# Ryan21wy/HSIMAE

Measured on AMD Instinct MI355X. Metric: HSI patches/sec (9x9x96, mask 75%) pretrain fwd+bwd, higher is better.
Workload: dtype bf16; 1 GPU; HSIMAE-Base pretrain fwd+bwd, 9x9x96 cubes, per-GPU batch 4096, mask 0.75, bf16 MFMA operands / fp32 accumulate + residual; per_gpu_batch=4096, global_batch=4096, parallelism=dp1

## Files before the change

### hsimae_amd/_lib.py

```python
from __future__ import annotations

import ctypes as C
import os

HERE = os.path.dirname(os.path.abspath(__file__))
LIB_PATH = os.environ.get("HSIMAE_LIB") or os.path.join(HERE, "libhsimae_hip.so")

i32, i64, f32, vp = C.c_int32, C.c_int64, C.c_float, C.c_void_p


class Config(C.Structure):
    _fields_ = [("bands", i32), ("embed_dim", i32), ("depth", i32), ("s_depth", i32), ("num_heads", i32),
                ("dec_dim", i32), ("dec_depth", i32), ("dec_heads", i32), ("hidden", i32), ("dec_hidden", i32),
                ("norm_pix_loss", i32), ("precision", i32)]


class IO(C.Structure):
    _fields_ = [("x", vp), ("sn", i64), ("sb", i64), ("sh", i64), ("sw", i64),
                ("N", i32), ("len_t", i32), ("len_l", i32),
                ("noise1", vp), ("noise2", vp), ("params", vp), ("wpk", vp),
                ("workspace", vp), ("workspace_bytes", i64),
                ("grad_scale", f32), ("want_recons", i32),
                ("loss", vp), ("pred_img", vp), ("mask_img", vp), ("mask", vp),
                ("ids_keep", vp), ("ids_restore", vp), ("latent", vp), ("pred", vp), ("drop_scale", vp),
# ... 87 lines not shown
class SceneParams(C.Structure):
    _fields_ = [("scene", vp), ("scene_f64", i32), ("H", i32), ("W", i32), ("C", i32),
                ("p0", i64), ("pixels", vp), ("N", i32),
                ("out", vp), ("sn", i64), ("sb", i64), ("sh", i64), ("sw", i64)]


class SceneBatchParams(C.Structure):
    _fields_ = [("scene", vp), ("scene_f64", i32), ("H", i32), ("W", i32), ("C", i32),
                ("items", vp), ("N", i32), ("n_items", i64), ("pixels", vp), ("labels", vp), ("flips", vp),
                ("out", vp), ("sn", i64), ("sb", i64), ("sh", i64), ("sw", i64), ("y", vp), ("bad", vp)]


class GwpcaParams(C.Structure):
    _fields_ = [("scene", vp), ("scene_f64", i32), ("H", i32), ("W", i32), ("C", i32), ("nc", i32), ("group", i32), ("whiten", i32),
                ("minmax", vp), ("mean", vp), ("lambda_", vp), ("proj", vp), ("group_off", vp)]


class ClsParams(C.Structure):
    _fields_ = [("logits", vp), ("ld", i32), ("targets", vp), ("N", i32), ("C", i32), ("ignore_index", i64), ("first", i32),
                ("loss", vp), ("n_valid", vp), ("dlogits", vp), ("ldd", i32), ("pred", vp), ("bad", vp), ("workspace", vp)]


class ClassProbParams(C.Structure):
    _fields_ = [("logits", vp), ("ld", i32), ("N", i32), ("C", i32), ("first", i32), ("view", i32), ("n_views", i32),
                ("acc", vp), ("lda", i32), ("H", i32), ("W", i32), ("p0", i64), ("pixels", vp),
                ("label_map", vp), ("conf_map", vp), ("margin_map", vp), ("probs", vp), ("ldp", i32)]


class RowNormalizeParams(C.Structure):
    _fields_ = [("x", vp), ("ld", i32), ("N", i32), ("D", i32), ("out", vp), ("ldo", i32), ("norms", vp)]
# ... 68 lines not shown
    "hsimae_dec_block_fwd": (C.c_int, [C.POINTER(DecBlockWeights), vp, vp, vp, vp, vp, i32, i32, i32, vp]),
    "hsimae_dec_block_bwd": (C.c_int, [C.POINTER(DecBlockWeights), C.POINTER(DecBlockGrads), vp, vp, vp, vp, vp, vp, vp, i32, i32, vp, vp]),
    "hsimae_attn_fwd": (C.c_int, [C.POINTER(AttnParams), vp]),
    "hsimae_attn_bwd": (C.c_int, [C.POINTER(AttnParams), vp]),
    "hsimae_attn_block_fwd": (C.c_int, [C.POINTER(AttnBlockWeights), vp, vp, vp, vp, vp, vp, vp, i32, i32, i32, i32, i32, i32, vp]),
    "hsimae_attn_block_bwd": (C.c_int, [C.POINTER(AttnBlockWeights), vp, vp, vp, vp, vp, vp, vp, vp, vp, vp, vp, vp, i32, i32, i32,
                                        i32, i32, i32, i32, vp]),
    "hsimae_wgrad": (C.c_int, [C.POINTER(WgradParams), vp]),
    "hsimae_wgrad_msplit": (i32, [i32, i64]),
    "hsimae_ln_bwd": (C.c_int, [C.POINTER(LnBwdParams), vp]),
    "hsimae_ln_fwd": (C.c_int, [vp, vp, vp, vp, i32, i32, vp]),
    "hsimae_assemble_fwd": (C.c_int, [C.POINTER(AssembleParams), vp]),
    "hsimae_assemble_bwd": (C.c_int, [C.POINTER(AssembleParams), vp]),
    "hsimae_loss_partials": (C.c_int, [i32, i32]),
    "hsimae_loss": (C.c_int, [C.POINTER(LossParams), vp]),
    "hsimae_adamw_step": (C.c_int, [vp, vp, vp, vp, vp, i64, f32, f32, f32, f32, f32, i32, vp]),
    "hsimae_grad_norm": (C.c_int, [C.POINTER(GradSeg), i32, f32, i32, i32, f32, f32, vp, vp, vp]),
    "hsimae_adamw_step_ctl": (C.c_int, [vp, vp, vp, vp, vp, i32, i64, f32, f32, f32, f32, f32, vp, vp]),
    "hsimae_adamw_step_groups": (C.c_int, [vp, vp, vp, vp, vp, i32, i64, C.POINTER(AdamWGroup), i32, f32, f32, f32, i32, vp, vp]),
    "hsimae_lamb_step": (C.c_int, [vp, vp, vp, vp, vp, i32, i64, vp, i32, i32, C.POINTER(AdamWGroup), i32, f32, f32, f32, f32, i32,
                                   vp, vp, vp, vp, vp]),
    "hsimae_ema_update": (C.c_int, [vp, vp, i64, C.c_double, i32, i32, vp, vp]),
    "hsimae_ema_swap": (C.c_int, [vp, vp, i64, vp]),
    "hsimae_cube_gather": (C.c_int, [C.POINTER(CubeParams), vp]),
    "hsimae_scene_windows": (C.c_int, [C.POINTER(SceneParams), vp]),
    "hsimae_class_argmax": (C.c_int, [C.POINTER(SceneParams), vp, i32, i32, i32, vp, vp]),
    "hsimae_scene_batch": (C.c_int, [C.POINTER(SceneBatchParams), vp]),
    "hsimae_gwpca_workspace_bytes": (i64, [C.POINTER(GwpcaParams)]),
    "hsimae_gwpca_fit": (C.c_int, [C.POINTER(GwpcaParams), vp, vp]),
    "hsimae_gwpca_apply": (C.c_int, [C.POINTER(GwpcaParams), vp, i32, vp]),
# ... 77 lines not shown
```

### hsimae_amd/build.py

```python
from __future__ import annotations

import os
import subprocess
import sys
from concurrent.futures import ThreadPoolExecutor

HERE = os.path.dirname(os.path.abspath(__file__))
CSRC = os.path.join(HERE, "csrc")
LIB = os.path.join(HERE, "libhsimae_hip.so")
UNITS = ["gemm", "attn", "attn_wide", "wgrad", "elem", "pack", "fused_dec", "fused_enc", "loader", "scene", "gwpca", "cls", "clip", "lamb", "ema", "prob", "knn", "api"]
HIPCC = os.environ.get("HIPCC", "/opt/rocm/bin/hipcc")
BASE_FLAGS = ["--offload-arch=gfx950", "-O3", "-fPIC", "-std=c++17", "-Wno-unused-value", "-fvisibility=hidden"]
FLAGS = BASE_FLAGS + os.environ.get("HSIMAE_HIPCC_EXTRA", "").split()


def flags_hash(flags: list[str]) -> str:
    import hashlib
    return hashlib.sha256(" ".join(flags).encode()).hexdigest()[:16]


def unit_flags(unit: str, flags: list[str]) -> list[str]:
    if unit != "api":
        return list(flags)
    return list(flags) + [f"-DHS_BUILD_FLAGS_HASH=0x{flags_hash(flags)}ULL", f"-DHS_BUILD_DEFAULT_FLAGS={int(flags == BASE_FLAGS)}",
                          f"-DHS_KERNEL_SOURCE_HASH=0x{kernel_source_hash()}ULL"]
# ... 100 lines not shown
```

### hsimae_amd/csrc/api.hip

```cpp
#include "common.h"
#include "kernels.h"
#include "plan.h"
#include <vector>
#include <algorithm>
#include <cstring>
#include <cstdlib>
#include <mutex>
#include <unordered_map>
#include <initializer_list>

using namespace hsplan;

namespace {

#define CK(expr) do { int _e = (expr); if (_e) return _e; } while (0)
#define CK0(expr) do { int _e0 = (expr); if (_e0) return _e0; } while (0)

inline hipStream_t S(void* s) { return reinterpret_cast<hipStream_t>(s); }
struct BlkP : BlockW {
    struct I8 { const uint8_t* w; const uint8_t* s; } qkv8, p8, w1_8, w3_8, w2_8, qkvT8, pT8, w13T8, w2T8;
};

BlkP resolve(const BlkOff& o, const BlkW& w, const float* P, const hs_bf16* wpk, const WLayout& WL, int h) {
    const float* fbase = reinterpret_cast<const float*>(wpk + WL.bf16_elems);
// ... 17 lines not shown
    if (!off("HSIMAE_FUSED_DEC")) b |= SC_FUSED_DEC;
    if (!off("HSIMAE_DEC_SPLIT")) b |= SC_DEC_SPLIT;
    if (one("HSIMAE_FP8_UNFUSED")) b |= SC_FP8_UNFUSED;
    if (!off("HSIMAE_FUSED_MLP")) b |= SC_FUSED_MLP;
    if (!off("HSIMAE_FUSED_ATTN_BLOCK")) b |= SC_ATTN_BLOCK;
    if (!off("HSIMAE_FUSED_ATTN_BLOCK256")) b |= SC_ATTN_BLOCK256;
    if (!off("HSIMAE_FUSED_ATTN_BLOCK_BWD")) b |= SC_ATTN_BLOCK_BWD;
    if (!off("HSIMAE_FUSED_PROJ_BWD")) b |= SC_PROJ_BWD;
    if (!off("HSIMAE_FUSED_LNBWD")) b |= SC_LNBWD;
    if (!off("HSIMAE_FUSED_LNBWD_512")) b |= SC_LNBWD_512;
    if (!off("HSIMAE_ATTN_BWD_RECOMPUTE")) b |= SC_RECOMPUTE;
    if (!off("HSIMAE_WGRAD_SLAB")) b |= SC_WGRAD_SLAB;
    if (!off("HSIMAE_DEC_SLAB")) b |= SC_DEC_SLAB;
    if (!off("HSIMAE_WGRAD_PLANAR")) b |= SC_PLANAR;
    if (!off("HSIMAE_FUSED_ATTN_BLOCK256_BWD")) b |= SC_ATTN_BLOCK256_BWD;
    return b;
}
struct SchedRec { uint32_t enc = 0, dec = 0; bool has_enc = false, has_dec = false; uint64_t gen = 0; };
std::mutex g_sched_mu;
std::unordered_map<const void*, SchedRec> g_sched;
uint64_t g_sched_gen = 0;
void record_sched(const void* ws, bool enc, bool dec, uint32_t bits) {
    std::lock_guard<std::mutex> lk(g_sched_mu);
    if (g_sched.size() > 4096 && g_sched.find(ws) == g_sched.end()) {
        std::vector<uint64_t> gens;
        gens.reserve(g_sched.size());
        for (auto& kv : g_sched) gens.push_back(kv.second.gen);
        std::nth_element(gens.begin(), gens.begin() + gens.size() / 2, gens.end());
        const uint64_t cut = gens[gens.size() / 2];
        for (auto it = g_sched.begin(); it != g_sched.end();) it = it->second.gen < cut ? g_sched.erase(it) : std::next(it);
// ... 283 lines not shown
        if (!io->workspace || !io->params || !io->wpk) return HSIMAE_ENULL;
        if (reinterpret_cast<uintptr_t>(io->workspace) % 256) return HSIMAE_EALIGN;
        carve(c.g, c.N, c.K, reinterpret_cast<char*>(io->workspace), c.w);
        if (c.w.bytes > io->workspace_bytes) return HSIMAE_EDIMS;
    }
    return HSIMAE_OK;
}

BlockPlan enc_plan(const Ctx& c, uint32_t sc) {
    return plan_block(c.g.D, c.g.H, c.g.h, c.K, c.N, c.Me, enc_linears_fp8(c.g.prec, c.g.D, sc), sc);
}
BlockPlan dec_block_plan(const Ctx& c, uint32_t sc) {
    return plan_block(c.g.Dd, c.g.Hd, c.g.hdec, c.g.TL, c.N, c.Md, false, sc);
}

int decoder_stack_fwd(const Ctx& c, const hsimae_io* io, uint32_t sc, float* pred, hipStream_t s) {
    const Geo& g = c.g; const Ws& w = c.w; const float* P = io->params;
    AssembleParams as; std::memset(&as, 0, sizeof(as));
    as.y = w.y; as.N = c.N; as.K = c.K; as.TL = g.TL; as.Dd = g.Dd; as.ld = g.Ddp; as.ids_restore = io->ids_restore; as.pos = P + c.L.dpos;
    as.yfull = w.yfull;
    CK(hs_assemble_fwd(as, s));
    const DecPlan dec = plan_dec(c.g.Dd, c.g.Hd, c.g.hdec, c.g.TL, sc);
    const BlockPlan lay = dec_block_plan(c, sc);
    const float* z = w.yfull;
    for (int i = 0; i < g.ddepth; ++i) {
        const BlkP bp = resolve(c.L.bd[i], c.W.bd[i], P, io->wpk, c.W, g.hdec);
        const BlkBuf& b = w.bd[i];
        if (!dec.fused) {
            CK(block_fwd(bp, lay, z, b, 0, 9, nullptr, s));
        } else if (dec.split) {
            CK(hs_dec_attn_fwd(z, b.x1, b.o, b.lse, c.N, g.TL, bp, s));
            CK(hs_enc_mlp_fwd(b.x1, nullptr, b.x2, (int)c.Md, g.Dd, bp, s));
        } else {
            CK(hs_dec_block_fwd(z, b.x1, b.x2, b.o, b.lse, c.N, g.TL, bp, s));
        }
        z = b.x2;
    }
    GemmParams p = gp();
    p.A = z; p.lda = g.Ddp; p.M = (int)c.Md; p.N = 80; p.K = g.Ddp; p.n_valid = 72; p.W = io->wpk + c.W.dp; p.bias = P + c.L.dpb;
    p.gamma = P + c.L.dnw; p.beta = P + c.L.dnb; p.u_out = w.zn; p.ldu = g.Ddp; p.out = pred; p.ldo = 72; p.ln_width = g.Dd;
    return hs_gemm(p, A_F32_LN, E_F32, s);
}

}

extern "C" unsigned hs_variant_bits_gemm();
extern "C" unsigned hs_variant_bits_attn();
extern "C" unsigned hs_variant_bits_attn_wide();
extern "C" unsigned hs_variant_bits_wgrad();
extern "C" unsigned hs_variant_bits_elem();
extern "C" unsigned hs_variant_bits_pack();
extern "C" unsigned hs_variant_bits_fused_dec();
extern "C" unsigned hs_variant_bits_fused_enc();
extern "C" unsigned hs_variant_bits_loader();
extern "C" unsigned hs_variant_bits_scene();
extern "C" unsigned hs_variant_bits_gwpca();
extern "C" unsigned hs_variant_bits_cls();
extern "C" unsigned hs_variant_bits_clip();
extern "C" unsigned hs_variant_bits_lamb();
extern "C" unsigned hs_variant_bits_ema();
extern "C" unsigned hs_variant_bits_prob();
extern "C" unsigned hs_variant_bits_knn();
#ifndef HS_KERNEL_SOURCE_HASH
#define HS_KERNEL_SOURCE_HASH 0ULL
#endif
#ifndef HS_BUILD_FLAGS_HASH
#define HS_BUILD_FLAGS_HASH 0ULL
#endif
#ifndef HS_BUILD_DEFAULT_FLAGS
#define HS_BUILD_DEFAULT_FLAGS 0
#endif

extern "C" {

int hsimae_version(void) { return HSIMAE_VERSION; }

int hsimae_build_info(hsimae_build_info_t* out) {
    if (!out) return HSIMAE_ENULL;
    out->abi_version = HSIMAE_VERSION;
    out->variant_bits = hs_variant_bits() | hs_variant_bits_gemm() | hs_variant_bits_attn() | hs_variant_bits_attn_wide() | hs_variant_bits_wgrad() | hs_variant_bits_elem() | hs_variant_bits_pack() | hs_variant_bits_fused_dec() | hs_variant_bits_fused_enc() | hs_variant_bits_loader() | hs_variant_bits_scene() | hs_variant_bits_gwpca() | hs_variant_bits_cls() | hs_variant_bits_clip() | hs_variant_bits_lamb() | hs_variant_bits_ema() | hs_variant_bits_prob() | hs_variant_bits_knn();
    out->kernel_source_hash = HS_KERNEL_SOURCE_HASH;
    out->flags_hash = HS_BUILD_FLAGS_HASH;
    out->default_flags = HS_BUILD_DEFAULT_FLAGS;
    out->reserved = 0;
    return HSIMAE_OK;
}
const char* hsimae_variant_name(int bit) {
    switch (bit) {
#define HS_X(b, name) case b: return #name;
        HS_VARIANT_TABLE(HS_X)
#undef HS_X
        default: return nullptr;
    }
}

// ... 42 lines not shown

struct DropRs { const float* a; const float* m; };
static DropRs drop_rs(const hsimae_io* io, int e, int64_t Me) {
    if (!io->drop_scale) return DropRs{nullptr, nullptr};
    const float* base = io->drop_scale + (int64_t)e * 2 * Me;
    return DropRs{base, base + Me};
}

static int forward_impl(const hsimae_config* cfg, const hsimae_io* io, void* stream, bool encoder_only) {
    Ctx c; CK(make_ctx(cfg, io, c, true));
    if (!io->x || !io->noise1 || !io->noise2 || !io->mask || !io->ids_keep || !io->ids_restore) return HSIMAE_ENULL;
    if (encoder_only ? !io->latent : !io->loss) return HSIMAE_ENULL;
    if (!encoder_only && io->want_recons && (!io->pred_img || !io->mask_img)) return HSIMAE_ENULL;
    hipStream_t s = S(stream);
    const Geo& g = c.g; const float* P = io->params; const Ws& w = c.w;
    const uint32_t sc = sched_from_env();
    record_sched(io->workspace, true, !encoder_only, sc);
    const BlockPlan enc = enc_plan(c, sc);

    MaskParams m; m.noise1 = io->noise1; m.noise2 = io->noise2; m.N = c.N; m.T = g.T; m.L = 9; m.len_t = c.len_t;
    m.len_l = c.len_l; m.ids_keep = io->ids_keep; m.ids_restore = io->ids_restore; m.mask = io->mask;
    CK(hs_mask(m, s));
    PatchParams pp; pp.x = io->x; pp.sn = io->sn; pp.sb = io->sb; pp.sh = io->sh; pp.sw = io->sw; pp.N = c.N; pp.T = g.T;
    pp.K = c.K; pp.ids_keep = io->ids_keep; pp.out = w.a_pe; pp.pos_ids = nullptr;
    CK(hs_patch_gather(pp, s));
    GemmParams p = gp();
    p.A = w.a_pe; p.lda = 96; p.M = (int)c.Me; p.N = g.Dp; p.K = 96; p.n_valid = g.D; p.W = io->wpk + c.W.pe; p.bias = P + c.L.peb;
    p.pos = P + c.L.pos; p.ids = io->ids_keep; p.ldpos = g.D; p.out = w.x0; p.ldo = g.Dp;
    CK(hs_gemm(p, A_BF16, E_POS_F32, s));

    const float* x = w.x0;
// ... 25 lines not shown
    }
    for (int i = 0; i < g.nfus; ++i) {
        BlkP bp = resolve(c.L.bf[i], c.W.bf[i], P, io->wpk, c.W, g.h);
        const DropRs rf = drop_rs(io, (g.has_axis ? 2 * g.sdepth : 0) + i, c.Me);
        CK(block_fwd(bp, enc, x, w.bf[i], 0, c.len_l, nullptr, s, rf.a, rf.m));
        x = w.bf[i].x2;
    }
    if (encoder_only) {
        CK(hs_ln_fwd(x, P + c.L.nw, P + c.L.nb, io->latent, (int)c.Me, g.D, s, g.Dp, g.D));
        return HSIMAE_OK;
    }
    p = gp();
    p.A = x; p.lda = g.Dp; p.M = (int)c.Me; p.N = g.Ddp; p.K = g.Dp; p.n_valid = g.Dd; p.W = io->wpk + c.W.de; p.bias = P + c.L.deb;
    p.gamma = P + c.L.nw; p.beta = P + c.L.nb; p.u_out = w.lat; p.ldu = g.Dp; p.out = w.y; p.ldo = g.Ddp; p.ln_width = g.D;
    CK(hs_gemm(p, A_F32_LN, E_F32, s));
    CK(decoder_stack_fwd(c, io, sc, w.pred, s));
    LossParams lp; std::memset(&lp, 0, sizeof(lp));
    const float sum_mask = (float)((int64_t)c.N * (g.TL - c.K));
    lp.x = io->x; lp.sn = io->sn; lp.sb = io->sb; lp.sh = io->sh; lp.sw = io->sw; lp.N = c.N; lp.T = g.T; lp.pred = w.pred;
    lp.mask = io->mask; lp.norm_pix = g.norm_pix; lp.inv_scale = io->grad_scale / (72.f * sum_mask); lp.partial = w.partial;
    lp.loss = io->loss; lp.sum_mask = sum_mask; lp.dpred = w.dpred;
    lp.pred_img = io->want_recons ? io->pred_img : nullptr; lp.mask_img = io->want_recons ? io->mask_img : nullptr;
    CK(hs_loss(lp, s));
    if (io->pred) CK((int)hipMemcpyAsync(io->pred, w.pred, c.Md * 72 * 4, hipMemcpyDeviceToDevice, s));
    if (io->latent) CK(hs_ln_fwd(x, P + c.L.nw, P + c.L.nb, io->latent, (int)c.Me, g.D, s, g.Dp, g.D));
    return HSIMAE_OK;
}

int hsimae_forward(const hsimae_config* cfg, const hsimae_io* io, void* stream) { return forward_impl(cfg, io, stream, false); }
int hsimae_encode(const hsimae_config* cfg, const hsimae_io* io, void* stream) { return forward_impl(cfg, io, stream, true); }

int hsimae_decode(const hsimae_config* cfg, const hsimae_io* io, const float* latent, float* pred, void* stream) {
    Ctx c; CK(make_ctx(cfg, io, c, true));
    if (!latent || !pred || !io->ids_restore) return HSIMAE_ENULL;
    hipStream_t s = S(stream);
    const Geo& g = c.g; const float* P = io->params; const Ws& w = c.w;
    const uint32_t sc = sched_from_env();
    record_sched(io->workspace, false, true, sc);
    GemmParams p = gp();
    const float* lat_in = latent;
    if (g.Dp != g.D) {
        CK((int)hipMemcpy2DAsync(w.G2, (size_t)g.Dp * 4, latent, (size_t)g.D * 4, (size_t)g.D * 4, (size_t)c.Me, hipMemcpyDeviceToDevice, s));
        lat_in = w.G2;
    }
    p.A = lat_in; p.lda = g.Dp; p.M = (int)c.Me; p.N = g.Ddp; p.K = g.Dp; p.n_valid = g.Dd; p.W = io->wpk + c.W.de; p.bias = P + c.L.deb;
    p.out = w.y; p.ldo = g.Ddp;
    CK(hs_gemm(p, A_F32, E_F32, s));
    CK(hs_rows_to_bf16(lat_in, w.lat, c.Me, g.Dp, nullptr, s));
    return decoder_stack_fwd(c, io, sc, pred, s);
}

static int encoder_backward(const Ctx& c, const hsimae_io* io, float* grads, hipStream_t s, Emitter& emit, uint32_t sc) {
// ... 35 lines not shown
        }
        if (!per_block) {
            for (int i = g.sdepth - 1; i >= 0; --i) CK(emit(L.b2[i].n1w, L.b2[i].end, s));
            for (int i = g.sdepth - 1; i >= 0; --i) CK(emit(L.b1[i].n1w, L.b1[i].end, s));
        }
    }
    CK(wgrad_one(w.G0, true, g.Dp, w.a_pe, 96, g.D, 72, c.Me, (g.D + 127) / 128, grads, L.pew, L.peb, io->det_acc, s));
    CK(emit(0, L.peb + g.D, s));
    return HSIMAE_OK;
}

static int decoder_backward(const Ctx& c, const hsimae_io* io, float* grads, hipStream_t s, Emitter& emit, uint32_t sc) {
    const Geo& g = c.g; const float* P = io->params; const Ws& w = c.w; const PLayout& L = c.L;
    const float* zlast = w.bd[g.ddepth - 1].x2;
    GemmParams p = gp();
    p.A = w.dpred; p.lda = 96; p.M = (int)c.Md; p.N = g.Ddp; p.K = 96; p.n_valid = g.Dd; p.W = io->wpk + c.W.dpT; p.out = w.du; p.ldo = g.Ddp;
    CK(hs_gemm(p, A_BF16, E_F32, s));
    CK(wgrad_one(w.dpred, false, 96, w.zn, g.Ddp, 72, g.Dd, c.Md, 1, grads, L.dpw, L.dpb, io->det_acc, s));
    LnBwdParams l; std::memset(&l, 0, sizeof(l));
    l.du = w.du; l.x = zlast; l.gamma = P + L.dnw; l.dres = nullptr; l.dx = w.G0; l.dgamma = grads + L.dnw; l.dbeta = grads + L.dnb;
    l.M = (int)c.Md; l.d = g.Dd; l.ld = g.Ddp; l.det_base = grads; l.det_acc = io->det_acc;
    CK(hs_ln_bwd(l, s));
    CK(emit(L.dnw, L.total, s));

    const DecPlan dec = plan_dec(c.g.Dd, c.g.Hd, c.g.hdec, c.g.TL, sc);
    const BlockPlan lay = dec_block_plan(c, sc);
    for (int i = g.ddepth - 1; i >= 0; --i) {
        BlkP bp = resolve(L.bd[i], c.W.bd[i], P, io->wpk, c.W, g.hdec);
        const float* xin = (i == 0) ? w.yfull : w.bd[i - 1].x2;
        if (dec.fused) {
            DecBlockBwd d;
            d.x = xin; d.x1 = w.bd[i].x1; d.dy = w.G0; d.dx1_tmp = w.G1; d.dx = w.G0; d.o = w.bd[i].o; d.lse = w.bd[i].lse;
            d.nsamples = c.N; d.Ts = g.TL; d.slab = dec.slab ? w.slab : nullptr;
            CK(hs_dec_block_bwd(bp, dec_grads(grads, L.bd[i], HsDet{grads, reinterpret_cast<long long*>(io->det_acc)}), d, s));
        } else {
            CK(block_bwd(bp, lay, L.bd[i], grads, xin, w.bd[i], 0, 9, w.G0, w.sc, w.G0, 0, s, 1, nullptr, nullptr, io->det_acc));
        }
// ... 270 lines not shown
}
int hsimae_lamb_step(float* params, const float* grads, float* exp_avg, float* exp_avg_sq, const uint8_t* group,
                     int32_t group_uniform, int64_t n, const hsimae_lamb_tensor* tensors, int32_t ntensors, int32_t nchunks,
                     const hsimae_adamw_group* table, int32_t ngroups, float beta1, float beta2, float eps, float trust_clip,
                     int32_t always_adapt, double* partials, float* ratios, int32_t* bad, const hsimae_clip_ctl* ctl, void* stream) {
    return hs_lamb_step(params, grads, exp_avg, exp_avg_sq, group, group_uniform, n, tensors, ntensors, nchunks, table, ngroups, beta1,
                        beta2, eps, trust_clip, always_adapt, partials, ratios, bad, ctl, S(stream));
}
int hsimae_ema_update(float* ema, const float* params, int64_t n, double decay, int32_t warmup, int32_t step,
                      const hsimae_clip_ctl* ctl, void* stream) {
    return hs_ema_update(ema, params, n, decay, warmup, step, ctl, S(stream));
}
int hsimae_ema_swap(float* a, float* b, int64_t n, void* stream) { return hs_ema_swap(a, b, n, S(stream)); }
int hsimae_loss_partials(int32_t N, int32_t T) { return hs_loss_partials(N, T); }
int hsimae_loss(const hsimae_loss_params* p, void* stream) { return p ? hs_loss(*p, S(stream)) : HSIMAE_ENULL; }

}
```

### hsimae_amd/csrc/kernels.h

```cpp
#pragma once
#include "common.h"
#include "../../include/hsimae_hip.h"

enum AKind { A_BF16 = HSIMAE_A_BF16, A_F32 = HSIMAE_A_F32, A_F32_LN = HSIMAE_A_F32_LN };
enum Epi { E_BF16 = HSIMAE_E_BF16, E_F32 = HSIMAE_E_F32, E_RES_F32 = HSIMAE_E_RES_F32,
           E_POS_F32 = HSIMAE_E_POS_F32, E_SWIGLU = HSIMAE_E_SWIGLU, E_SWIGLU_BWD = HSIMAE_E_SWIGLU_BWD,
           E_LN_BWD = HSIMAE_E_LN_BWD };

typedef hsimae_gemm_params GemmParams;
typedef hsimae_pack_desc PackDesc;
typedef hsimae_attn_params AttnParams;
typedef hsimae_wgrad_task WgradTask;
typedef hsimae_wgrad_params WgradParams;
typedef hsimae_lnbwd_params LnBwdParams;
typedef hsimae_mask_params MaskParams;
typedef hsimae_patch_params PatchParams;
typedef hsimae_assemble_params AssembleParams;
typedef hsimae_loss_params LossParams;
typedef hsimae_cube_params CubeParams;
typedef hsimae_scene_params SceneParams;

int hs_gemm(const GemmParams& p, int akind, int epi, hipStream_t s);
int hs_gemm_tiled(const GemmParams& p, int akind, int epi, int bm, int kc, hipStream_t s);
int hs_pack(const PackDesc* descs_dev, int ndesc, int max_elems, hipStream_t s);
int hs_attn_fwd(const AttnParams& p, hipStream_t s);
int hs_attn_bwd(const AttnParams& p, hipStream_t s);
int hs_wgrad(const WgradParams& p, hipStream_t s);
int hs_ln_bwd(const LnBwdParams& p, hipStream_t s);
int hs_ln_fwd(const float* x, const float* gamma, const float* beta, float* out, int M, int d, hipStream_t s, int ldx = 0, int ldo = 0);
int hs_mask(const MaskParams& p, hipStream_t s);
int hs_patch_gather(const PatchParams& p, hipStream_t s);
int hs_assemble_fwd(const AssembleParams& p, hipStream_t s);
int hs_assemble_bwd(const AssembleParams& p, hipStream_t s);
int hs_loss(const LossParams& p, hipStream_t s);
int hs_loss_partials(int N, int T);
int hs_cube_gather(const CubeParams& p, hipStream_t s);
int hs_scene_windows(const SceneParams& p, hipStream_t s);
int hs_class_argmax(const SceneParams& p, const float* logits, int ld, int num_class, int first, int64_t* map, hipStream_t s);
int hs_scene_batch(const hsimae_scene_batch_params& p, hipStream_t s);
int64_t hs_gwpca_workspace_bytes(const hsimae_gwpca_params& p);
int hs_gwpca_fit(const hsimae_gwpca_params& p, void* workspace, hipStream_t s);
int hs_gwpca_apply(const hsimae_gwpca_params& p, void* out, int out_f64, hipStream_t s);
int64_t hs_cls_workspace_bytes(int N);
int hs_cls_loss(const hsimae_cls_params& p, hipStream_t s);
int hs_cls_grad_scale(const float* src, const float* scale, float* dst, int64_t n, hipStream_t s);
int hs_confusion(const int64_t* gt, const int64_t* pred, int64_t n, int C, int64_t* cm, int32_t* bad, hipStream_t s);
int hs_confusion_map(const int64_t* gt_map, const int64_t* mask_map, const int64_t* pred_map, int64_t* masked, int64_t n, int C,
                     int64_t* cm, int32_t* bad, hipStream_t s);
int hs_scores(const int64_t* cm, int C, double* out, hipStream_t s);
int hs_class_prob(const hsimae_class_prob_params& p, hipStream_t s);
// ... 70 lines not shown
```

### hsimae_amd/csrc/plan.h

```cpp
#pragma once
#include "../../include/hsimae_hip.h"
#include <algorithm>
#include <cstdint>
#include <cstdlib>
#include <cstring>
#include <vector>

namespace hsplan {

typedef hsimae_pack_desc PackDesc;
constexpr int LOSS_ROWS_PER_WG = 32;
inline int loss_partials(int N, int T) {
    const int64_t M = (int64_t)N * T * 9;
    return (int)std::max<int64_t>((M + LOSS_ROWS_PER_WG - 1) / LOSS_ROWS_PER_WG, N);
}

inline int rup(int x, int m) { return (x + m - 1) / m * m; }

struct BlkOff { int64_t n1w, n1b, qw, qb, kw, kb, vw, vb, pw, pb, n2w, n2b, w1w, w1b, w2w, w2b, w3w, w3b, end; };

struct Geo {
    int B, T, TL, D, H, hd, h, hp, Dd, Hd, hdd, hdec, hpd, depth, sdepth, nfus, ddepth, norm_pix, prec;
    int Dp, Ddp;
    bool has_axis, has_fus;
// ... 372 lines not shown
    SC_FUSED_DEC = 1u << 0,
    SC_DEC_SPLIT = 1u << 1,
    SC_FP8_UNFUSED = 1u << 2,
    SC_FUSED_MLP = 1u << 3,
    SC_ATTN_BLOCK = 1u << 4,
    SC_ATTN_BLOCK256 = 1u << 5,
    SC_ATTN_BLOCK_BWD = 1u << 6,
    SC_PROJ_BWD = 1u << 7,
    SC_LNBWD = 1u << 8,
    SC_LNBWD_512 = 1u << 9,
    SC_RECOMPUTE = 1u << 10,
    SC_WGRAD_SLAB = 1u << 11,
    SC_DEC_SLAB = 1u << 12,
    SC_PLANAR = 1u << 13,
    SC_ATTN_BLOCK256_BWD = 1u << 14,
};

constexpr int kAttnTile = 16, kAttnMaxTs = 2 * kAttnTile;
constexpr int kAttn128D = 128, kAttn128Heads = 8;
constexpr int kAttn256D = 256, kAttn256Heads = 16;
constexpr bool mlp_shape(int d, int hp) {
    return (d == 128 && hp == 352) || (d == 256 && hp == 704) || (d == 64 && hp == 192);
}
constexpr int kDecD = 64, kDecHeads = 8, kDecHp = 192, kDecMinTs = 16, kDecMaxTs = 112;
inline bool attn128_fusable(int d, int heads, int Ts) { return d == kAttn128D && heads == kAttn128Heads && Ts <= kAttnMaxTs; }
inline bool attn256_fusable(int d, int heads, int Ts, int nsamples) {
    return d == kAttn256D && heads == kAttn256Heads && Ts >= 1 && Ts <= kAttnMaxTs && (int64_t)nsamples * Ts * 3 * kAttn256D < (1ll << 31);
}
inline bool mlp_fusable(int d, int hidden) { return mlp_shape(d, rup(hidden, 32)); }
inline bool dec_fusable(int d, int heads, int hidden, int Ts) {
    return d == kDecD && heads == kDecHeads && rup(hidden, 32) == kDecHp && hidden % 4 == 0 && Ts <= kDecMaxTs && Ts >= kDecMinTs;
}

inline bool enc_linears_fp8(int model_prec, int D, uint32_t sc) {
    return model_prec == HSIMAE_PREC_FP8 && (D >= 512 || (sc & SC_FP8_UNFUSED));
}

enum AttnFwd { ATTN_FWD_LAYERED, ATTN_FWD_BLK128, ATTN_FWD_BLK256 };
enum AttnBwd { ATTN_BWD_LAYERED, ATTN_BWD_BLK128, ATTN_BWD_BLK128_RECOMPUTE, ATTN_BWD_BLK256 };
enum LnBwd { LN_SEPARATE, LN_GEMM_EPILOGUE, LN_IN_KERNEL };
struct BlockPlan {
    int d, dp, heads, h, hp, Ts, nsamples; int64_t M;
    AttnFwd attn_fwd;
    bool save_qkv;
// ... 82 lines not shown
```

### include/hsimae_hip.h

```cpp
#ifndef HSIMAE_HIP_H
#define HSIMAE_HIP_H
#include <stdint.h>

#ifdef __HIPCC__
typedef __bf16 hs_bf16;
#else
typedef uint16_t hs_bf16;
#endif

#ifdef __cplusplus
extern "C" {
#endif
#pragma GCC visibility push(default)

#define HSIMAE_OK 0
#define HSIMAE_EDIMS (-1)
#define HSIMAE_EUNSUPPORTED (-2)
#define HSIMAE_EALIGN (-3)
#define HSIMAE_ENULL (-4)
#define HSIMAE_ENOFORWARD (-5)

#define HSIMAE_VERSION 108
int hsimae_version(void);
typedef struct {
// ... 339 lines not shown

#define HSIMAE_LAMB_CHUNK 4096
typedef struct { int64_t off; int64_t n; int32_t chunk0; int32_t reserved; } hsimae_lamb_tensor;
int hsimae_lamb_step(float* params, const float* grads, float* exp_avg, float* exp_avg_sq, const uint8_t* group,
                     int32_t group_uniform, int64_t n, const hsimae_lamb_tensor* tensors , int32_t ntensors,
                     int32_t nchunks, const hsimae_adamw_group* table , int32_t ngroups, float beta1, float beta2, float eps,
                     float trust_clip , int32_t always_adapt, double* partials ,
                     float* ratios , int32_t* bad , const hsimae_clip_ctl* ctl ,
                     void* stream);

#define HSIMAE_EMA_MAX_GRID 2048
int hsimae_ema_update(float* ema, const float* params, int64_t n, double decay, int32_t warmup, int32_t step,
                      const hsimae_clip_ctl* ctl , void* stream);
int hsimae_ema_swap(float* a, float* b, int64_t n, void* stream);

#pragma GCC visibility pop
#ifdef __cplusplus
}
#endif
#endif
```

Measured before the change: 273,200 patches/s.

## Fuse decoder head backward: dgrad, weight grad, and LayerNorm backward in one kernel

Adds a single kernel that computes the decoder prediction-head backward for dec_dim 64. It recomputes the LayerNorm output from the last decoder activation, runs the data-gradient MFMA, accumulates weight and bias grads from LDS-staged tiles, and does LayerNorm backward in place. Because the normalized output is recomputed, the forward head GEMM no longer writes it out. This removes three launches plus the round trips of the du and zn intermediates. In exchange it recomputes LN statistics and adds a persistent-grid kernel with atomic gradient accumulation.

```diff
diff --git a/hsimae_amd/_lib.py b/hsimae_amd/_lib.py
--- a/hsimae_amd/_lib.py
+++ b/hsimae_amd/_lib.py
@@ -125,6 +125,11 @@
 class GwpcaParams(C.Structure):
     _fields_ = [("scene", vp), ("scene_f64", i32), ("H", i32), ("W", i32), ("C", i32), ("nc", i32), ("group", i32), ("whiten", i32),
                 ("minmax", vp), ("mean", vp), ("lambda_", vp), ("proj", vp), ("group_off", vp)]
+
+
+class DecHeadBwdParams(C.Structure):
+    _fields_ = [("dpred", vp), ("z", vp), ("ldz", i32), ("gamma", vp), ("beta", vp), ("ln_width", i32), ("WT", vp),
+                ("dx", vp), ("dW", vp), ("db", vp), ("dgamma", vp), ("dbeta", vp), ("M", i64), ("det_base", vp), ("det_acc", vp)]
 
 
 class ClsParams(C.Structure):
@@ -223,6 +228,8 @@
     "hsimae_assemble_bwd": (C.c_int, [C.POINTER(AssembleParams), vp]),
     "hsimae_loss_partials": (C.c_int, [i32, i32]),
     "hsimae_loss": (C.c_int, [C.POINTER(LossParams), vp]),
+    "hsimae_head_fusable": (C.c_int, [i32]),
+    "hsimae_dec_head_bwd": (C.c_int, [C.POINTER(DecHeadBwdParams), vp]),
     "hsimae_adamw_step": (C.c_int, [vp, vp, vp, vp, vp, i64, f32, f32, f32, f32, f32, i32, vp]),
     "hsimae_grad_norm": (C.c_int, [C.POINTER(GradSeg), i32, f32, i32, i32, f32, f32, vp, vp, vp]),
     "hsimae_adamw_step_ctl": (C.c_int, [vp, vp, vp, vp, vp, i32, i64, f32, f32, f32, f32, f32, vp, vp]),
diff --git a/hsimae_amd/build.py b/hsimae_amd/build.py
--- a/hsimae_amd/build.py
+++ b/hsimae_amd/build.py
@@ -8,7 +8,7 @@
 HERE = os.path.dirname(os.path.abspath(__file__))
 CSRC = os.path.join(HERE, "csrc")
 LIB = os.path.join(HERE, "libhsimae_hip.so")
-UNITS = ["gemm", "attn", "attn_wide", "wgrad", "elem", "pack", "fused_dec", "fused_enc", "loader", "scene", "gwpca", "cls", "clip", "lamb", "ema", "prob", "knn", "api"]
+UNITS = ["gemm", "attn", "attn_wide", "wgrad", "elem", "pack", "fused_dec", "fused_enc", "dec_head", "loader", "scene", "gwpca", "cls", "clip", "lamb", "ema", "prob", "knn", "api"]
 HIPCC = os.environ.get("HIPCC", "/opt/rocm/bin/hipcc")
 BASE_FLAGS = ["--offload-arch=gfx950", "-O3", "-fPIC", "-std=c++17", "-Wno-unused-value", "-fvisibility=hidden"]
 FLAGS = BASE_FLAGS + os.environ.get("HSIMAE_HIPCC_EXTRA", "").split()
diff --git a/hsimae_amd/csrc/api.hip b/hsimae_amd/csrc/api.hip
--- a/hsimae_amd/csrc/api.hip
+++ b/hsimae_amd/csrc/api.hip
@@ -55,6 +55,7 @@
     if (!off("HSIMAE_DEC_SLAB")) b |= SC_DEC_SLAB;
     if (!off("HSIMAE_WGRAD_PLANAR")) b |= SC_PLANAR;
     if (!off("HSIMAE_FUSED_ATTN_BLOCK256_BWD")) b |= SC_ATTN_BLOCK256_BWD;
+    if (!off("HSIMAE_FUSED_HEAD")) b |= SC_FUSED_HEAD;
     return b;
 }
 struct SchedRec { uint32_t enc = 0, dec = 0; bool has_enc = false, has_dec = false; uint64_t gen = 0; };
@@ -368,6 +369,8 @@
     return plan_block(c.g.Dd, c.g.Hd, c.g.hdec, c.g.TL, c.N, c.Md, false, sc);
 }
 
+uint32_t dec_sched(const Geo& g, uint32_t sc) { return head_fusable(g.Dd, g.Ddp) ? sc : (sc & ~SC_FUSED_HEAD); }
+
 int decoder_stack_fwd(const Ctx& c, const hsimae_io* io, uint32_t sc, float* pred, hipStream_t s) {
     const Geo& g = c.g; const Ws& w = c.w; const float* P = io->params;
     AssembleParams as; std::memset(&as, 0, sizeof(as));
@@ -392,7 +395,7 @@
     }
     GemmParams p = gp();
     p.A = z; p.lda = g.Ddp; p.M = (int)c.Md; p.N = 80; p.K = g.Ddp; p.n_valid = 72; p.W = io->wpk + c.W.dp; p.bias = P + c.L.dpb;
-    p.gamma = P + c.L.dnw; p.beta = P + c.L.dnb; p.u_out = w.zn; p.ldu = g.Ddp; p.out = pred; p.ldo = 72; p.ln_width = g.Dd;
+    p.gamma = P + c.L.dnw; p.beta = P + c.L.dnb; p.u_out = (sc & SC_FUSED_HEAD) ? nullptr : w.zn; p.ldu = g.Ddp; p.out = pred; p.ldo = 72; p.ln_width = g.Dd;
     return hs_gemm(p, A_F32_LN, E_F32, s);
 }
 
@@ -406,6 +409,7 @@
 extern "C" unsigned hs_variant_bits_pack();
 extern "C" unsigned hs_variant_bits_fused_dec();
 extern "C" unsigned hs_variant_bits_fused_enc();
+extern "C" unsigned hs_variant_bits_dec_head();
 extern "C" unsigned hs_variant_bits_loader();
 extern "C" unsigned hs_variant_bits_scene();
 extern "C" unsigned hs_variant_bits_gwpca();
@@ -432,7 +436,7 @@
 int hsimae_build_info(hsimae_build_info_t* out) {
     if (!out) return HSIMAE_ENULL;
     out->abi_version = HSIMAE_VERSION;
-    out->variant_bits = hs_variant_bits() | hs_variant_bits_gemm() | hs_variant_bits_attn() | hs_variant_bits_attn_wide() | hs_variant_bits_wgrad() | hs_variant_bits_elem() | hs_variant_bits_pack() | hs_variant_bits_fused_dec() | hs_variant_bits_fused_enc() | hs_variant_bits_loader() | hs_variant_bits_scene() | hs_variant_bits_gwpca() | hs_variant_bits_cls() | hs_variant_bits_clip() | hs_variant_bits_lamb() | hs_variant_bits_ema() | hs_variant_bits_prob() | hs_variant_bits_knn();
+    out->variant_bits = hs_variant_bits() | hs_variant_bits_gemm() | hs_variant_bits_attn() | hs_variant_bits_attn_wide() | hs_variant_bits_wgrad() | hs_variant_bits_elem() | hs_variant_bits_pack() | hs_variant_bits_fused_dec() | hs_variant_bits_fused_enc() | hs_variant_bits_dec_head() | hs_variant_bits_loader() | hs_variant_bits_scene() | hs_variant_bits_gwpca() | hs_variant_bits_cls() | hs_variant_bits_clip() | hs_variant_bits_lamb() | hs_variant_bits_ema() | hs_variant_bits_prob() | hs_variant_bits_knn();
     out->kernel_source_hash = HS_KERNEL_SOURCE_HASH;
     out->flags_hash = HS_BUILD_FLAGS_HASH;
     out->default_flags = HS_BUILD_DEFAULT_FLAGS;
@@ -505,7 +509,7 @@
     if (!encoder_only && io->want_recons && (!io->pred_img || !io->mask_img)) return HSIMAE_ENULL;
     hipStream_t s = S(stream);
     const Geo& g = c.g; const float* P = io->params; const Ws& w = c.w;
-    const uint32_t sc = sched_from_env();
+    const uint32_t sc = dec_sched(g, sched_from_env());
     record_sched(io->workspace, true, !encoder_only, sc);
     const BlockPlan enc = enc_plan(c, sc);
 
@@ -561,9 +565,9 @@
     p.A = x; p.lda = g.Dp; p.M = (int)c.Me; p.N = g.Ddp; p.K = g.Dp; p.n_valid = g.Dd; p.W = io->wpk + c.W.de; p.bias = P + c.L.deb;
     p.gamma = P + c.L.nw; p.beta = P + c.L.nb; p.u_out = w.lat; p.ldu = g.Dp; p.out = w.y; p.ldo = g.Ddp; p.ln_width = g.D;
     CK(hs_gemm(p, A_F32_LN, E_F32, s));
+    const float sum_mask = (float)((int64_t)c.N * (g.TL - c.K));
     CK(decoder_stack_fwd(c, io, sc, w.pred, s));
     LossParams lp; std::memset(&lp, 0, sizeof(lp));
-    const float sum_mask = (float)((int64_t)c.N * (g.TL - c.K));
     lp.x = io->x; lp.sn = io->sn; lp.sb = io->sb; lp.sh = io->sh; lp.sw = io->sw; lp.N = c.N; lp.T = g.T; lp.pred = w.pred;
     lp.mask = io->mask; lp.norm_pix = g.norm_pix; lp.inv_scale = io->grad_scale / (72.f * sum_mask); lp.partial = w.partial;
     lp.loss = io->loss; lp.sum_mask = sum_mask; lp.dpred = w.dpred;
@@ -582,7 +586,7 @@
     if (!latent || !pred || !io->ids_restore) return HSIMAE_ENULL;
     hipStream_t s = S(stream);
     const Geo& g = c.g; const float* P = io->params; const Ws& w = c.w;
-    const uint32_t sc = sched_from_env();
+    const uint32_t sc = dec_sched(g, sched_from_env());
     record_sched(io->workspace, false, true, sc);
     GemmParams p = gp();
     const float* lat_in = latent;
@@ -648,6 +652,13 @@
     const Geo& g = c.g; const float* P = io->params; const Ws& w = c.w; const PLayout& L = c.L;
     const float* zlast = w.bd[g.ddepth - 1].x2;
     GemmParams p = gp();
+    if (sc & SC_FUSED_HEAD) {
+        hsimae_dec_head_bwd_params h; std::memset(&h, 0, sizeof(h));
+        h.dpred = w.dpred; h.z = zlast; h.ldz = g.Ddp; h.gamma = P + L.dnw; h.beta = P + L.dnb; h.ln_width = g.Dd; h.WT = io->wpk + c.W.dpT;
+        h.dx = w.G0; h.dW = grads + L.dpw; h.db = grads + L.dpb; h.dgamma = grads + L.dnw; h.dbeta = grads + L.dnb; h.M = c.Md;
+        h.det_base = io->det_acc ? grads : nullptr; h.det_acc = io->det_acc;
+        CK(hs_dec_head_bwd(h, s));
+    } else {
     p.A = w.dpred; p.lda = 96; p.M = (int)c.Md; p.N = g.Ddp; p.K = 96; p.n_valid = g.Dd; p.W = io->wpk + c.W.dpT; p.out = w.du; p.ldo = g.Ddp;
     CK(hs_gemm(p, A_BF16, E_F32, s));
     CK(wgrad_one(w.dpred, false, 96, w.zn, g.Ddp, 72, g.Dd, c.Md, 1, grads, L.dpw, L.dpb, io->det_acc, s));
@@ -655,6 +666,7 @@
     l.du = w.du; l.x = zlast; l.gamma = P + L.dnw; l.dres = nullptr; l.dx = w.G0; l.dgamma = grads + L.dnw; l.dbeta = grads + L.dnb;
     l.M = (int)c.Md; l.d = g.Dd; l.ld = g.Ddp; l.det_base = grads; l.det_acc = io->det_acc;
     CK(hs_ln_bwd(l, s));
+    }
     CK(emit(L.dnw, L.total, s));
 
     const DecPlan dec = plan_dec(c.g.Dd, c.g.Hd, c.g.hdec, c.g.TL, sc);
@@ -955,5 +967,7 @@
 int hsimae_ema_swap(float* a, float* b, int64_t n, void* stream) { return hs_ema_swap(a, b, n, S(stream)); }
 int hsimae_loss_partials(int32_t N, int32_t T) { return hs_loss_partials(N, T); }
 int hsimae_loss(const hsimae_loss_params* p, void* stream) { return p ? hs_loss(*p, S(stream)) : HSIMAE_ENULL; }
-
-}
+int hsimae_head_fusable(int32_t dec_dim) { return head_fusable(dec_dim, rup(dec_dim, 32)) ? 1 : 0; }
+int hsimae_dec_head_bwd(const hsimae_dec_head_bwd_params* p, void* stream) { return p ? hs_dec_head_bwd(*p, S(stream)) : HSIMAE_ENULL; }
+
+}
diff --git a/hsimae_amd/csrc/dec_head.hip b/hsimae_amd/csrc/dec_head.hip
--- /dev/null
+++ b/hsimae_amd/csrc/dec_head.hip
@@ -0,0 +1,187 @@
+#include "common.h"
+#include "kernels.h"
+#include "plan.h"
+#include <algorithm>
+
+namespace {
+
+using hsplan::kHeadD;
+static_assert(kHeadD == 64, "rows of two 32-deep k-steps / four 16-column tiles");
+
+__device__ __forceinline__ void wave_lds_fence() { asm volatile("s_waitcnt lgkmcnt(0)" ::: "memory"); }
+
+constexpr int HB_LDT = 72;
+constexpr int HB_LDX = 68;
+
+__global__ __launch_bounds__(256, 2) void dec_head_bwd_kernel(hsimae_dec_head_bwd_params p) {
+    __shared__ __attribute__((aligned(16))) bf16_t ZNT[64 * HB_LDT];
+    __shared__ __attribute__((aligned(16))) bf16_t DPT[80 * HB_LDT];
+    __shared__ __attribute__((aligned(16))) float XH[64 * HB_LDX];
+    __shared__ float RS[64];
+    __shared__ float red[2][4][64];
+    const int tid = threadIdx.x, lane = tid & 63, wave = __builtin_amdgcn_readfirstlane(tid >> 6);
+    const int c = lane & 15, g = lane >> 4;
+    const int c8 = (lane & 7) * 8, rl = lane >> 3;
+
+    bf16x8 wt[4][3];
+#pragma unroll
+    for (int nt = 0; nt < 4; ++nt)
+#pragma unroll
+        for (int ks = 0; ks < 3; ++ks) wt[nt][ks] = *reinterpret_cast<const bf16x8*>(p.WT + ((size_t)(nt * 3 + ks) * 64 + lane) * 8);
+    float gm8[8], bt8[8], gmc[4];
+#pragma unroll
+    for (int e = 0; e < 8; ++e) { gm8[e] = p.gamma[c8 + e]; bt8[e] = p.beta[c8 + e]; }
+#pragma unroll
+    for (int nt = 0; nt < 4; ++nt) gmc[nt] = p.gamma[nt * 16 + c];
+    const float invd = 1.f / (float)kHeadD;
+
+    f32x4 dw[5];
+    float dbp[5], dgam[4], dbet[4];
+#pragma unroll
+    for (int i = 0; i < 5; ++i) { dw[i] = f32x4{0.f, 0.f, 0.f, 0.f}; dbp[i] = 0.f; }
+#pragma unroll
+    for (int i = 0; i < 4; ++i) { dgam[i] = 0.f; dbet[i] = 0.f; }
+
+    const int64_t npanels = (p.M + 63) / 64;
+    for (int64_t panel = blockIdx.x; panel < npanels; panel += gridDim.x) {
+        const int64_t r0 = panel * 64 + wave * 16;
+        bf16x8 a[3];
+#pragma unroll
+        for (int ks = 0; ks < 3; ++ks)
+            a[ks] = r0 + c < p.M ? *reinterpret_cast<const bf16x8*>(p.dpred + (r0 + c) * 96 + ks * 32 + g * 8) : zero8();
+        float f[2][8];
+#pragma unroll
+        for (int i = 0; i < 2; ++i) {
+            const int64_t row = min(r0 + rl + 8 * i, p.M - 1);
+            ld8(p.z + row * kHeadD + c8, f[i]);
+        }
+#pragma unroll
+        for (int i = 0; i < 2; ++i) {
+            const int rr = wave * 16 + rl + 8 * i;
+            const bool rv = r0 + rl + 8 * i < p.M;
+            float sm = 0.f;
+#pragma unroll
+            for (int e = 0; e < 8; ++e) sm += f[i][e];
+            sm = lanes_sum<8>(sm);
+            const float mean = sm * invd;
+            float q = 0.f;
+#pragma unroll
+            for (int e = 0; e < 8; ++e) { const float dl = f[i][e] - mean; q += dl * dl; }
+            q = lanes_sum<8>(q);
+            const float rstd = rsqrtf(q * invd + 1e-5f);
+            float xh[8];
+#pragma unroll
+            for (int e = 0; e < 8; ++e) {
+                xh[e] = rv ? (f[i][e] - mean) * rstd : 0.f;
+                const float y = (f[i][e] - mean) * rstd * gm8[e] + bt8[e];
+                ZNT[(c8 + e) * HB_LDT + rr] = rv ? (bf16_t)y : (bf16_t)0.f;
+            }
+            *reinterpret_cast<float4*>(XH + rr * HB_LDX + c8) = make_float4(xh[0], xh[1], xh[2], xh[3]);
+            *reinterpret_cast<float4*>(XH + rr * HB_LDX + c8 + 4) = make_float4(xh[4], xh[5], xh[6], xh[7]);
+            if ((lane & 7) == 0) RS[rr] = rstd;
+        }
+#pragma unroll
+        for (int ks = 0; ks < 3; ++ks)
+            if (ks < 2 || g < 2) {
+#pragma unroll
+                for (int j = 0; j < 8; ++j) DPT[(ks * 32 + g * 8 + j) * HB_LDT + wave * 16 + c] = a[ks][j];
+            }
+        f32x4 du[4];
+#pragma unroll
+        for (int nt = 0; nt < 4; ++nt) {
+            du[nt] = f32x4{0.f, 0.f, 0.f, 0.f};
+#pragma unroll
+            for (int ks = 0; ks < 3; ++ks) du[nt] = mfma16(a[ks], wt[nt][ks], du[nt]);
+        }
+        wave_lds_fence();
+#pragma unroll
+        for (int r = 0; r < 4; ++r) {
+            const int rr = wave * 16 + 4 * g + r;
+            const float rstd = RS[rr];
+            float xh[4], tt[4], sa = 0.f, sb = 0.f;
+#pragma unroll
+            for (int nt = 0; nt < 4; ++nt) {
+                xh[nt] = XH[rr * HB_LDX + nt * 16 + c];
+                tt[nt] = du[nt][r] * gmc[nt];
+                sa += tt[nt];
+                sb += tt[nt] * xh[nt];
+                dgam[nt] += du[nt][r] * xh[nt];
+                dbet[nt] += du[nt][r];
+            }
+            sa = lanes_sum<16>(sa) * invd;
+            sb = lanes_sum<16>(sb) * invd;
+#pragma unroll
+            for (int nt = 0; nt < 4; ++nt) XH[rr * HB_LDX + nt * 16 + c] = rstd * (tt[nt] - sa - xh[nt] * sb);
+        }
+        wave_lds_fence();
+#pragma unroll
+        for (int i = 0; i < 2; ++i) {
+            const int rr = wave * 16 + rl + 8 * i;
+            const int64_t row = r0 + rl + 8 * i;
+            if (row < p.M) {
+                const float4 v0 = *reinterpret_cast<const float4*>(XH + rr * HB_LDX + c8);
+                const float4 v1 = *reinterpret_cast<const float4*>(XH + rr * HB_LDX + c8 + 4);
+                float* op = p.dx + row * kHeadD + c8;
+                *reinterpret_cast<float4*>(op) = v0;
+                *reinterpret_cast<float4*>(op + 4) = v1;
+            }
+        }
+        lds_barrier();
+#pragma unroll
+        for (int ks = 0; ks < 2; ++ks) {
+            const bf16x8 b = *reinterpret_cast<const bf16x8*>(ZNT + (wave * 16 + c) * HB_LDT + ks * 32 + g * 8);
+#pragma unroll
+            for (int ft = 0; ft < 5; ++ft) {
+                const bf16x8 af = *reinterpret_cast<const bf16x8*>(DPT + (ft * 16 + c) * HB_LDT + ks * 32 + g * 8);
+                dw[ft] = mfma16(af, b, dw[ft]);
+                if (wave == 0) {
+#pragma unroll
+                    for (int j = 0; j < 8; ++j) dbp[ft] += bf2f(af[j]);
+                }
+            }
+        }
+        lds_barrier();
+    }
+
+    const HsDet det{p.det_base, reinterpret_cast<long long*>(p.det_acc)};
+#pragma unroll
+    for (int ft = 0; ft < 5; ++ft)
+#pragma unroll
+        for (int r = 0; r < 4; ++r) {
+            const int fr = ft * 16 + 4 * g + r;
+            if (fr < 72) hs_gadd(det, p.dW + fr * kHeadD + wave * 16 + c, dw[ft][r]);
+        }
+    if (wave == 0) {
+#pragma unroll
+        for (int ft = 0; ft < 5; ++ft) {
+            const float v = rows_sum(dbp[ft]);
+            if (g == 0 && ft * 16 + c < 72) hs_gadd(det, p.db + ft * 16 + c, v);
+        }
+    }
+#pragma unroll
+    for (int nt = 0; nt < 4; ++nt) {
+        const float vg = rows_sum(dgam[nt]), vb = rows_sum(dbet[nt]);
+        if (g == 0) { red[0][wave][nt * 16 + c] = vg; red[1][wave][nt * 16 + c] = vb; }
+    }
+    __syncthreads();
+    if (tid < 128) {
+        const int which = tid >> 6, col = tid & 63;
+        const float v = (red[which][0][col] + red[which][1][col]) + (red[which][2][col] + red[which][3][col]);
+        hs_gadd(det, (which ? p.dbeta : p.dgamma) + col, v);
+    }
+}
+
+}
+
+int hs_dec_head_bwd(const hsimae_dec_head_bwd_params& p, hipStream_t s) {
+    if (!p.dpred || !p.z || !p.gamma || !p.beta || !p.WT || !p.dx || !p.dW || !p.db || !p.dgamma || !p.dbeta) return HS_ENULL;
+    if ((p.det_base == nullptr) != (p.det_acc == nullptr)) return HS_ENULL;
+    if (p.M < 0) return HS_EDIMS;
+    if (!hsplan::head_fusable(p.ln_width, p.ldz)) return HS_EUNSUPPORTED;
+    if (p.M == 0) return HS_OK;
+    const int64_t npanels = (p.M + 63) / 64;
+    hipLaunchKernelGGL(dec_head_bwd_kernel, dim3((unsigned)std::min<int64_t>(npanels, hsplan::kHeadBwdGrid)), dim3(256), 0, s, p);
+    return (int)hipGetLastError();
+}
+
+HS_UNIT_VARIANT_BITS(dec_head)
diff --git a/hsimae_amd/csrc/kernels.h b/hsimae_amd/csrc/kernels.h
--- a/hsimae_amd/csrc/kernels.h
+++ b/hsimae_amd/csrc/kernels.h
@@ -34,6 +34,7 @@
 int hs_assemble_bwd(const AssembleParams& p, hipStream_t s);
 int hs_loss(const LossParams& p, hipStream_t s);
 int hs_loss_partials(int N, int T);
+int hs_dec_head_bwd(const hsimae_dec_head_bwd_params& p, hipStream_t s);
 int hs_cube_gather(const CubeParams& p, hipStream_t s);
 int hs_scene_windows(const SceneParams& p, hipStream_t s);
 int hs_class_argmax(const SceneParams& p, const float* logits, int ld, int num_class, int first, int64_t* map, hipStream_t s);
diff --git a/hsimae_amd/csrc/plan.h b/hsimae_amd/csrc/plan.h
--- a/hsimae_amd/csrc/plan.h
+++ b/hsimae_amd/csrc/plan.h
@@ -410,6 +410,7 @@
     SC_DEC_SLAB = 1u << 12,
     SC_PLANAR = 1u << 13,
     SC_ATTN_BLOCK256_BWD = 1u << 14,
+    SC_FUSED_HEAD = 1u << 15,
 };
 
 constexpr int kAttnTile = 16, kAttnMaxTs = 2 * kAttnTile;
@@ -424,6 +425,9 @@
     return d == kAttn256D && heads == kAttn256Heads && Ts >= 1 && Ts <= kAttnMaxTs && (int64_t)nsamples * Ts * 3 * kAttn256D < (1ll << 31);
 }
 inline bool mlp_fusable(int d, int hidden) { return mlp_shape(d, rup(hidden, 32)); }
+constexpr int kHeadD = 64;
+constexpr int kHeadBwdGrid = 512;
+inline bool head_fusable(int Dd, int Ddp) { return Dd == kHeadD && Ddp == kHeadD; }
 inline bool dec_fusable(int d, int heads, int hidden, int Ts) {
     return d == kDecD && heads == kDecHeads && rup(hidden, 32) == kDecHp && hidden % 4 == 0 && Ts <= kDecMaxTs && Ts >= kDecMinTs;
 }
diff --git a/include/hsimae_hip.h b/include/hsimae_hip.h
--- a/include/hsimae_hip.h
+++ b/include/hsimae_hip.h
@@ -377,6 +377,17 @@
                       const hsimae_clip_ctl* ctl , void* stream);
 int hsimae_ema_swap(float* a, float* b, int64_t n, void* stream);
 
+typedef struct {
+    const hs_bf16* dpred; const float* z; int32_t ldz;
+    const float* gamma; const float* beta; int32_t ln_width;
+    const hs_bf16* WT;
+    float* dx; float* dW; float* db; float* dgamma; float* dbeta;
+    int64_t M;
+    const float* det_base; int64_t* det_acc;
+} hsimae_dec_head_bwd_params;
+int hsimae_head_fusable(int32_t dec_dim);
+int hsimae_dec_head_bwd(const hsimae_dec_head_bwd_params* p, void* stream);
+
 #pragma GCC visibility pop
 #ifdef __cplusplus
 }
```

After: 276,300 patches/s, median of 5. About the same (+1.1%).
